# danielSanchezQ/dkg

Hardware: AMD Instinct MI355X
Metric: verified shares/sec (whole node) at n=1024,t=511; full-ceremony wall time (higher is better)
Workload: dtype u32 (GF(2^255-19), Z_l); 1 GPU; one DKG ceremony n=1024, t=511 (share gen + round-2/4 checks + finalise); n=1024, t=511, parallelism=single GPU, verify_streams=2, rounds_2_4_fused=True, degree_split=4, recombination=short lattice multipliers, recombination_addends=affine Niels, stepping_additions=dedicated (complete redo where exceptional)

## Files before the change

dkg_amd/__init__.py:

```python
from ._lib import (ACCEPT, COMPLAINT_IGNORED, COMPLAINT_NO_PHASE3, COMPLAINT_NOT_OWNED, MISSING, REJECT, SELF,
                   SKIPPED, DkgError, lib)
from .api import (Backend, BatchProvenResult, BatchResult, MultiBackend, CeremonyResult, ProvenResult, Environment, ceremony_batch_device,
                  ceremony_batch_full_device, ceremony_batch_verify, ceremony_batch_verify_full, ceremony_batch_verify_full_proven,
                  ceremony_batch_verify_proven, comb_geometry, dealer_coefficients, enc_randomness, env_check, key_comb_choice, merge_verdicts,
                  packed_row_words, pair_eval_shape, receiver_plan, receiver_plan_constants, seat_disclosures, seat_enc_digits, seat_eval_shape, seat_finalise_status, seat_pack,
                  shard_range, shard_rows, split_multipliers)

__all__ = ["Backend", "MultiBackend", "Environment", "CeremonyResult", "BatchResult", "DkgError", "dealer_coefficients", "env_check",
           "ceremony_batch_device", "ceremony_batch_verify", "ceremony_batch_full_device", "ceremony_batch_verify_full", "enc_randomness", "split_multipliers", "lib",
           "shard_range", "shard_rows", "packed_row_words", "key_comb_choice",
           "ceremony_batch_verify_proven", "ceremony_batch_verify_full_proven", "BatchProvenResult",
           "ACCEPT", "REJECT", "SELF", "SKIPPED", "MISSING", "ProvenResult", "COMPLAINT_IGNORED", "COMPLAINT_NO_PHASE3",
           "COMPLAINT_NOT_OWNED", "merge_verdicts", "receiver_plan", "receiver_plan_constants", "pair_eval_shape",
           "comb_geometry", "seat_pack", "seat_finalise_status", "seat_disclosures", "seat_enc_digits", "seat_eval_shape"]
```

dkg_amd/_lib.py:

```python
import ctypes
import os
import sys

HERE = os.path.dirname(os.path.abspath(__file__))
LIB_PATH = os.environ.get("DKG_AMD_LIB", os.path.join(HERE, "libdkg_amd.so"))

DKG_OK = 0
DKG_E_ARG = -1
DKG_E_DECODE = -2
DKG_E_DEVICE = -3
DKG_E_NOMEM = -4
REJECT, ACCEPT, SELF, SKIPPED, MISSING = 0, 1, 2, 3, 4
FIN_OK, FIN_R2_ERROR, FIN_R4_ERROR, FIN_PHASE4_ERROR, FIN_INSUFFICIENT, FIN_PANIC = 0, 1, 2, 3, 4, 5
COMPLAINT_IGNORED, COMPLAINT_NO_PHASE3 = 4, 5
COMPLAINT_NOT_OWNED = -2

_lib = None


class DkgError(RuntimeError):
    def __init__(self, code, msg=""):
        self.code = code
        names = {DKG_E_ARG: "DKG_E_ARG", DKG_E_DECODE: "DKG_E_DECODE", DKG_E_DEVICE: "DKG_E_DEVICE",
                 DKG_E_NOMEM: "DKG_E_NOMEM"}
# ... 211 lines not shown
    L.dkg_dealer_coeffs.argtypes = [u8p, ctypes.c_uint32, sz, sz, sz, p, p]
    L.dkg_scalar_sum_device.argtypes = [p, sz, sz, p, p, p]
    L.dkg_point_sum_device.argtypes = [p, sz, p, p, p]
    L.dkg_share_gen_device.argtypes = [p, sz, sz, sz, p, p, p, p, p, p]
    L.dkg_ceremony_shard_recon_device.argtypes = [p, sz, sz, sz, sz, u8p, u8p, u8p, u8p, p, p,
                                                  ctypes.POINTER(ctypes.c_int32)]
    L.dkg_finalise_parties.argtypes = [p, sz, sz, u8p, u8p, u8p, u8p, u8p, u8p, u8p, p, p, p]
    L.dkg_shard_range.argtypes = [sz, sz, sz, ctypes.POINTER(sz), ctypes.POINTER(sz)]
    L.dkg_shard_range.restype = None
    L.dkg_shard_rows.argtypes = [sz, sz]
    L.dkg_shard_rows.restype = sz
    L.dkg_shard_combine_device.argtypes = [p, sz, sz, sz, p, p, p, p, ctypes.POINTER(ShardOutcome)]
    L.dkg_shard_combine_packed_device.argtypes = [p, sz, sz, sz, p, p, p, p, ctypes.POINTER(ShardOutcome)]
    L.dkg_fixed_base_windows.argtypes = []
    L.dkg_key_comb_windows.argtypes = []
    if hasattr(L, "dkg_comb_geometry"):
        L.dkg_ctx_set_comb_build.argtypes = [p, ctypes.c_int]
        L.dkg_ctx_last_comb_build.argtypes = [p]
        L.dkg_ctx_last_comb_build_ms.argtypes = [p]
        L.dkg_ctx_last_comb_build_ms.restype = ctypes.c_double
        L.dkg_comb_geometry.argtypes = [ctypes.c_int, ctypes.POINTER(ctypes.c_int), ctypes.POINTER(ctypes.c_int),
                                        ctypes.POINTER(ctypes.c_uint32), ctypes.POINTER(ctypes.c_uint32)]
        L.dkg_comb_entries.argtypes = [p, ctypes.c_int, u8p, ctypes.c_int, ctypes.c_uint32, ctypes.c_uint32, p]
    L.dkg_packed_row_words.argtypes = [sz]
    L.dkg_packed_row_words.restype = sz
    L.dkg_decisions_pack_device.argtypes = [p, sz, sz, sz, sz, p, p]
    L.dkg_shard_finalise_device.argtypes = [p, sz, sz, sz, p, p, u8p, ctypes.c_int, p, p, p]
    L.dkg_multi_create.argtypes = [ctypes.POINTER(ctypes.c_int), ctypes.c_int, ctypes.POINTER(p)]
    L.dkg_multi_destroy.argtypes = [p]
    L.dkg_multi_destroy.restype = None
    L.dkg_multi_size.argtypes = [p]
    L.dkg_multi_ctx.argtypes = [p, ctypes.c_int]
    L.dkg_multi_ctx.restype = p
    L.dkg_multi_last_error.argtypes = [p]
    L.dkg_multi_last_error.restype = ctypes.c_char_p
    L.dkg_multi_phase_ms.argtypes = [p, ctypes.c_char_p]
    L.dkg_multi_phase_ms.restype = ctypes.c_double
    L.dkg_multi_env_init.argtypes = [p, sz, sz, u8p, sz, p]
    L.dkg_multi_ceremony_run.argtypes = [p, sz, sz, u8p, u8p, ctypes.POINTER(CeremonyOut)]
    L.dkg_multi_ceremony_run_device.argtypes = [p, sz, sz, ctypes.POINTER(p), ctypes.POINTER(p),
                                                ctypes.POINTER(CeremonyOut)]
    L.dkg_multi_ceremony_verify.argtypes = [p, sz, sz, u8p, u8p, u8p, u8p, ctypes.POINTER(CeremonyOut)]
    L.dkg_multi_ceremony_run_full.argtypes = [p, sz, sz, u8p, u8p, u8p, u8p, u8p, ctypes.POINTER(CeremonyOut)]
    L.dkg_multi_ceremony_run_full_device.argtypes = [p, sz, sz, ctypes.POINTER(p), ctypes.POINTER(p), ctypes.POINTER(p),
                                                     u8p, u8p, ctypes.POINTER(CeremonyOut)]
    L.dkg_multi_ceremony_verify_full.argtypes = [p, sz, sz, u8p, u8p, u8p, u8p, u8p, ctypes.POINTER(CeremonyOut)]
# ... 19 lines not shown
    "dkg_shard_combine_packed_device", "dkg_packed_row_words", "dkg_fixed_base_windows", "dkg_key_comb_windows", "dkg_decisions_pack_device",
    "dkg_shard_finalise_device", "dkg_multi_create", "dkg_multi_destroy", "dkg_multi_size", "dkg_multi_ctx",
    "dkg_multi_last_error", "dkg_multi_phase_ms", "dkg_multi_env_init", "dkg_multi_ceremony_run",
    "dkg_multi_ceremony_run_device", "dkg_multi_ceremony_verify",
    "dkg_member_keys_batch", "dkg_encrypt_shares_batch", "dkg_decrypt_shares_batch", "dkg_ceremony_batch_full_device",
    "dkg_ceremony_batch_verify_full", "dkg_ctx_set_batch_full_chunk",
    "dkg_complaints_prove", "dkg_complaints_verify", "dkg_ctx_set_complaint_eval", "dkg_ceremony_verify_full_complaints",
    "dkg_complaints3_verify", "dkg_ceremony_verify_fetched_proven", "dkg_ceremony_verify_full_proven",
    "dkg_ceremony_batch_verify_proven", "dkg_ceremony_batch_verify_full_proven",
    "dkg_ceremony_shard_full_device", "dkg_ceremony_shard_verify_full_device", "dkg_ctx_set_key_comb",
    "dkg_ctx_last_key_comb", "dkg_key_comb_choice", "dkg_key_comb_constants", "dkg_multi_ceremony_run_full",
    "dkg_multi_ceremony_run_full_device", "dkg_multi_ceremony_verify_full",
    "dkg_ceremony_shard_verify_proven_device", "dkg_ceremony_shard_verify_full_proven_device",
    "dkg_ctx_last_complaint_eval", "dkg_shard_combine_proven_device",
    "dkg_multi_ceremony_verify_proven", "dkg_multi_ceremony_verify_full_proven",
    "dkg_receiver_plan_for", "dkg_receiver_plan_cost_us", "dkg_receiver_plan_constants", "dkg_ctx_set_receiver_chunk",
    "dkg_ctx_set_comb_build", "dkg_ctx_last_comb_build", "dkg_ctx_last_comb_build_ms", "dkg_comb_geometry", "dkg_comb_entries",
    "dkg_ctx_last_receiver_chunk", "dkg_pair_eval_shape", "dkg_commitment_eval_pairs", "dkg_commitment_eval", "dkg_verify_receivers", "dkg_party_round2",
    "dkg_seat_pack", "dkg_commitment_eval_seats", "dkg_verify_seats", "dkg_party_round2_seats",
    "dkg_complaints_verify_ceremonies", "dkg_complaints3_verify_ceremonies", "dkg_party_round3_seats", "dkg_finalise_seats",
    "dkg_seat_finalise_status",
    "dkg_party_round1_seats", "dkg_ctx_set_seat_deal", "dkg_ctx_last_seat_deal", "dkg_seat_enc_digits",
    "dkg_seat_eval_shape", "dkg_seat_eval_constants", "dkg_ctx_set_seat_eval", "dkg_ctx_last_seat_eval",
]
```

dkg_amd/api.py:

```python
import ctypes
from collections.abc import Sequence
from dataclasses import dataclass
from typing import List, Optional

from . import _lib
from ._lib import BatchOut, CeremonyOut, DkgError

CK_DEFAULT = b"Example of a shared string."


def _check(ctx, rc):
    if rc != _lib.DKG_OK:
        msg = _lib.lib().dkg_ctx_last_error(ctx).decode() if ctx else ""
        raise DkgError(rc, msg)


def env_check(threshold: int, nr_members: int) -> None:
    rc = _lib.lib().dkg_env_check(threshold, nr_members)
    if rc != _lib.DKG_OK:
        raise DkgError(rc, f"threshold {threshold} must be < (nr_members + 1) / 2 = {(nr_members + 1) // 2}")


def dealer_coefficients(master: bytes, ceremony: int, d0: int, D: int, t: int):
    N = t + 1
# ... 241 lines not shown
        arr = _carray(ctypes.c_uint32, M, xs)
        out = ctypes.create_string_buffer(32 * max(D * M, 1))
        _check(self._ctx, _lib.lib().dkg_poly_eval_batch(self._ctx, D, N, coeffs, M, arr, out))
        return out.raw[: 32 * D * M]

    def points_valid(self, points: bytes) -> bytes:
        count = len(points) // 32
        out = ctypes.create_string_buffer(max(count, 1))
        _check(self._ctx, _lib.lib().dkg_points_valid_batch(self._ctx, count, points, out))
        return out.raw[:count]

    def share_gen(self, a: bytes, b: bytes, D: int, n: int, t: int):
        N = t + 1
        E, A = ctypes.create_string_buffer(32 * D * N), ctypes.create_string_buffer(32 * D * N)
        s, sp = ctypes.create_string_buffer(32 * D * n), ctypes.create_string_buffer(32 * D * n)
        _check(self._ctx, _lib.lib().dkg_share_gen(self._ctx, D, n, t, a, b, E, A, s, sp))
        return E.raw, A.raw, s.raw, sp.raw

    def share_gen_device(self, D: int, n: int, t: int, d_a: int, d_b: int, d_E: Optional[int], d_A: Optional[int],
                         d_s: int, d_sp: int):
        vp = ctypes.c_void_p
        _check(self._ctx, _lib.lib().dkg_share_gen_device(self._ctx, D, n, t, vp(d_a), vp(d_b), vp(d_E), vp(d_A),
                                                           vp(d_s), vp(d_sp)))

    def verify_pairs(self, n: int, t: int, rnd: int, d0: int, d1: int, C: bytes, s: bytes,
                     s_prime: Optional[bytes] = None) -> bytes:
        dec = ctypes.create_string_buffer(max((d1 - d0) * n, 1))
        _check(self._ctx, _lib.lib().dkg_verify_pairs(self._ctx, n, t, rnd, d0, d1, C, s, s_prime, dec))
        return dec.raw[: (d1 - d0) * n]

    def verify_receiver(self, n: int, t: int, rnd: int, j: int, C: bytes, s_col: bytes,
                        sp_col: Optional[bytes] = None) -> bytes:
        dec = ctypes.create_string_buffer(max(n, 1))
        _check(self._ctx, _lib.lib().dkg_verify_receiver(self._ctx, n, t, rnd, j, C, s_col, sp_col, dec))
        return dec.raw[:n]

    def set_receiver_chunk(self, chunk: int = 0):
        _check(self._ctx, _lib.lib().dkg_ctx_set_receiver_chunk(self._ctx, chunk))

    def last_receiver_chunk(self) -> int:
        return _lib.lib().dkg_ctx_last_receiver_chunk(self._ctx)

    def commitment_eval(self, D: int, t: int, js: Sequence[int], C: bytes):
        M = len(js)
        arr = (ctypes.c_uint32 * max(M, 1))(*js)
        P = ctypes.create_string_buffer(max(32 * M * D, 1))
# ... 751 lines not shown
    v = [ctypes.c_uint32() for _ in range(4)]
    rc = _lib.lib().dkg_seat_pack(n, S, ja, ctypes.byref(v[0]), ctypes.byref(v[1]), ctypes.byref(v[2]), wave_of, slot_of,
                                  ctypes.byref(v[3]))
    if rc != _lib.DKG_OK:
        raise _lib.DkgError(rc, "seat_pack")
    return {"width": v[0].value, "per_wave": v[1].value, "tiles": v[2].value, "wave_of": list(wave_of[:S]),
            "slot_of": list(slot_of[:S]), "waves": v[3].value}


def seat_eval_shape(n: int, t: int, waves: int, x_max: int, chunk: int = 0) -> dict:
    v = [ctypes.c_uint32() for _ in range(3)]
    sb = ctypes.c_uint64()
    L = _lib.lib()
    rc = L.dkg_seat_eval_shape(n, t, waves, x_max, chunk, *[ctypes.byref(x) for x in v], ctypes.byref(sb))
    if rc != _lib.DKG_OK:
        raise _lib.DkgError(rc, "seat_eval_shape")
    c = (ctypes.c_double * 6)()
    L.dkg_seat_eval_constants(c)
    return {"chunk": v[0].value, "chunks": v[1].value, "stages": v[2].value, "scratch_bytes": sb.value,
            "constants": dict(zip(("launch_us", "op_latency_us", "lane_op_us", "serial_op_latency_us",
                                   "chunked_setup_us", "margin"), c))}


def seat_enc_digits(k: int) -> List[int]:
    if k < 0 or k >= 1 << 256:
        raise _lib.DkgError(_lib.DKG_E_ARG, "seat_enc_digits")
    d = (ctypes.c_int8 * 128)()
    w = ctypes.c_int(0)
    rc = _lib.lib().dkg_seat_enc_digits(k.to_bytes(32, "little"), d, ctypes.byref(w))
    if rc != _lib.DKG_OK:
        raise _lib.DkgError(rc, "seat_enc_digits")
    return list(d[: w.value])


def seat_finalise_status(n: int, t: int, p: int, qualified, reconstruct, points: Sequence[int], a_present=None,
                         r2_error: bool = False, r4_error: bool = False):
    mask = lambda x: None if x is None else bytes(bytearray(x))
    idx = ctypes.c_int32(-1)
    rc = _lib.lib().dkg_seat_finalise_status(n, t, p, mask(qualified), mask(reconstruct), mask(a_present),
                                             (ctypes.c_uint32 * max(n, 1))(*points), int(bool(r2_error)),
                                             int(bool(r4_error)), ctypes.byref(idx))
    if rc < 0:
        raise _lib.DkgError(rc, "seat_finalise_status")
    return rc, idx.value


# ... 242 lines not shown
```

dkg_amd/csrc/kernels_decl.inc:

```
namespace dkgk {

void decode_points(const uint32_t* comp, size_t count, uint32_t* ext, size_t stride, uint8_t* ok,
                   hipStream_t stream);
void place_position_major(const uint32_t* src, size_t sstride, size_t D, size_t N, size_t npad, uint32_t* out,
                          hipStream_t stream, int nseg = 1, int seg = 0, size_t L = 0, size_t pstride = 0);
void gather_points(const uint32_t* src, size_t sstride, size_t step, size_t k0, size_t count, uint32_t* dst,
                   size_t dstride, hipStream_t stream);
void decode_position_major(const uint32_t* comp, size_t D, size_t N, size_t npad, uint32_t* out, uint8_t* ok,
                           hipStream_t stream, int nseg = 1, int seg = 0, size_t L = 0, size_t pstride = 0);
void fill_identity(size_t S, uint32_t* out, hipStream_t stream);
void check_both(size_t ndealers, size_t nrecv, size_t dealer0, size_t dealer_base, size_t nmod, const uint32_t* s,
                const uint32_t* sp, const uint32_t* R, const uint32_t* tab_g, const uint32_t* tab_h,
                const uint8_t* dok, uint8_t* dec2, uint8_t* dec4, hipStream_t stream, const uint32_t* scale = nullptr,
                size_t j0 = 0, size_t jn = 0, uint32_t* acc = nullptr);
void encode_points(const uint32_t* ext, size_t stride, size_t count, uint32_t* comp, hipStream_t stream);
void build_comb(const uint32_t* ext, size_t stride, size_t e0, uint32_t* tab, hipStream_t stream, size_t count = 1);
void build_combw(const uint32_t* ext, size_t stride, size_t e0, uint32_t* tab, hipStream_t stream, size_t count = 1);

void commit_position_major(size_t D, size_t N, const uint32_t* a, const uint32_t* b, const uint32_t* tab_g,
                           const uint32_t* tab_h, uint32_t* out, size_t W, size_t L, size_t pstride, uint32_t* A0,
                           size_t A0stride, hipStream_t stream);
void commit(size_t count, const uint32_t* a, const uint32_t* b, const uint32_t* tab_g,
            const uint32_t* tab_h, uint32_t* A_ext, uint32_t* E_ext, hipStream_t stream, size_t stride = 0);
void share_eval(size_t D, size_t n, size_t N, const uint32_t* a, const uint32_t* b, uint32_t* s,
                uint32_t* sp, hipStream_t stream);
void poly_eval(size_t D, size_t N, const uint32_t* coeffs, size_t M, const uint32_t* xs, uint32_t* out,
               hipStream_t stream);

uint32_t* binomial(size_t width, size_t npad, size_t N, const uint32_t* C, uint32_t* e0, uint32_t* e1,
                   hipStream_t stream, size_t pieces = 1, size_t pstride = 0, size_t last_len = 0);
void binom_init(size_t width, size_t npad, size_t N, const uint32_t* C, uint32_t* e0, hipStream_t stream,
                size_t pieces = 1, size_t pstride = 0);
void binom_step(size_t r, size_t width, size_t npad, size_t N, const uint32_t* C, const uint32_t* in, uint32_t* out,
                hipStream_t stream, size_t pieces = 1, size_t pstride = 0, size_t last_len = 0,
                uint32_t* flags = nullptr, size_t col_base = 0, size_t dreal = 0, unsigned gw = 64,
                bool flag_any = false,
                bool nt = false,
                bool il = false);
void binomial_wave_redo(size_t width, size_t npad, size_t N, const uint32_t* C, uint32_t* e, hipStream_t stream,
                        size_t pieces, size_t pstride, size_t last_len, uint32_t* flags, size_t col_base,
                        size_t dreal, unsigned gw);
uint32_t* binomial_wave(size_t width, size_t npad, size_t N, const uint32_t* C, uint32_t* e, hipStream_t stream,
                        size_t pieces = 1, size_t pstride = 0, size_t last_len = 0, uint32_t* eT = nullptr,
                        bool prefetch = false, uint32_t* flags = nullptr, size_t col_base = 0, size_t dreal = 0,
                        unsigned gw = 64);
void binom_step_pair(size_t r, size_t width, size_t npad, size_t N, const uint32_t* C, const uint32_t* in,
                     uint32_t* out, hipStream_t stream, size_t pieces = 1, size_t pstride = 0, size_t last_len = 0);
void to_column_major(size_t width, size_t npad, size_t N, const uint32_t* e, uint32_t* eT, size_t pieces,
// ... 192 lines not shown
```

dkg_amd/csrc/runtime.hip:

```cpp
#include <hip/hip_runtime.h>

#include <cstdio>
#include <cstdlib>
#include <cstring>
#include <algorithm>
#include <array>
#include <iterator>
#include <map>
#include <memory>
#include <optional>
#include <string>
#include <thread>
#include <unordered_map>
#include <unordered_set>
#include <vector>

#include "../../include/dkg_amd.h"
#include "host_crypto.h"
#include "kernels.h"
#include "kernels_ilp.h"
#include "comb_build.h"
#include "seat_finalise.h"
#include "seat_deal.h"

// ... 9 lines not shown
  uint32_t* tab_hw = nullptr;
  uint8_t h[32] = {0};
  bool have_h = false;
  size_t threshold = 0, nr_members = 0;
  hipEvent_t ev[8] = {};
  struct PhaseMark {
    const char* tag;
    int phase;
  };
  std::vector<hipEvent_t> phase_pool;
  std::vector<PhaseMark> phase_marks;
  int receiver_chunk = 0;
  int last_receiver_chunk = 0;
  std::map<std::array<size_t, 4>, dkg_receiver_plan> recv_plans;
  std::map<std::array<size_t, 3>, std::vector<uint32_t>> pair_digits;
  static constexpr int MAX_SUB = 8;
  int nsub = 2;
  hipStream_t sub[MAX_SUB] = {};
  hipEvent_t fork = nullptr, join[MAX_SUB] = {};
  hipStream_t side = nullptr;
  hipEvent_t side_fork = nullptr, shares_done = nullptr, pub_done = nullptr;
  hipEvent_t terms_done = nullptr;
  bool shares_pending = false;
  bool overlap = true;
  int split = 0;
  std::vector<uint8_t> key_tabs_pk;
  std::vector<uint8_t> key_tabs16_pk;
  int key_comb = 0;
  int last_key_comb = 0;
  int seat_deal = 0;
  int last_seat_deal = 0;
  int seat_eval = 0, seat_eval_chunk = 0;
  int last_seat_eval = 0, last_seat_eval_chunk = 0;
  uint8_t fb_base[32] = {0};
  bool fb_valid = false;
  int comb_build = 0;
  int last_comb_build = 0;
  hipEvent_t cb_ev[2] = {};
  int binom_mode = 0;
  int step_mode = 0;
  int check_mode = 0;
  int fe_mode = 0;
  int verify_mode = 0;
  size_t vinv_N = 0;
  size_t fallback_rows = 0;
  int last_split = 1;
// ... 1222 lines not shown
struct Commitments {
  uint32_t *E, *A;
};
Commitments commitment_rows(dkg_ctx* ctx, size_t n, size_t N) {
  uint32_t* EA = buf<uint32_t>(ctx, "cer_EA", 32 * 2 * n * N);
  return {EA, EA + 8 * n * N};
}
Commitments upload_commitments(dkg_ctx* ctx, size_t n, size_t N, const uint8_t* E, const uint8_t* A) {
  const Commitments c = commitment_rows(ctx, n, N);
  h2d(ctx, c.E, E, 32 * n * N);
  h2d(ctx, c.A, A, 32 * n * N);
  return c;
}

void ceremony_times(dkg_ctx* ctx, dkg_ceremony_out* out, bool round1) {
  out->ms_round1 = round1 ? ev_ms(ctx, 0, 1) : 0.0;
  out->ms_round2 = ev_ms(ctx, 1, 2);
  out->ms_round3 = ev_ms(ctx, 2, 3);
  out->ms_round4 = ev_ms(ctx, 3, 4);
  out->ms_finalise = ev_ms(ctx, 4, 5);
  out->ms_total = ev_ms(ctx, 0, 5);
}

void round1_device(dkg_ctx* ctx, size_t D, size_t n, size_t t, const uint32_t* a, const uint32_t* b,
                   uint32_t* Ecomp, uint32_t* Acomp, uint32_t* s, uint32_t* sp, bool encode = true,
                   bool overlap_shares = false) {
  const size_t N = t + 1;
  uint32_t* Aext = buf<uint32_t>(ctx, "Aext", PTB * D * N);
  uint32_t* Eext = buf<uint32_t>(ctx, "Eext", PTB * D * N);
  if (overlap_shares) {
    HCK(hipEventRecord(ctx->side_fork, ctx->stream));
    HCK(hipStreamWaitEvent(ctx->side, ctx->side_fork, 0));
  }
  dkgk::commit(D * N, a, b, ctx->tab_gw, ctx->tab_hw, Aext, Eext, ctx->stream);
  if (encode) {
    dkgk::encode_points(Eext, D * N, D * N, Ecomp, ctx->stream);
    dkgk::encode_points(Aext, D * N, D * N, Acomp, ctx->stream);
  }
  if (overlap_shares) {
    dkgk::share_eval(D, n, N, a, b, s, sp, ctx->side);
    HCK(hipEventRecord(ctx->shares_done, ctx->side));
    ctx->shares_pending = true;
  } else {
    dkgk::share_eval(D, n, N, a, b, s, sp, ctx->stream);
  }
  check_launch(ctx);
}


struct SharesScope {
  dkg_ctx* ctx;
  explicit SharesScope(dkg_ctx* c) : ctx(c) {}
  ~SharesScope() {
    if (ctx->shares_pending) (void)hipStreamWaitEvent(ctx->stream, ctx->shares_done, 0);
    ctx->shares_pending = false;
  }
};

struct ExtScope {
  dkg_ctx* ctx;
  ExtScope(dkg_ctx* c, size_t D, size_t N) : ctx(c) {
    ctx->ext_E = buf<uint32_t>(ctx, "Eext", PTB * D * N);
    ctx->ext_A = buf<uint32_t>(ctx, "Aext", PTB * D * N);
    ctx->ext_stride = D * N;
  }
  ~ExtScope() {
    ctx->ext_E = ctx->ext_A = nullptr;
    ctx->ext_stride = 0;
  }
};

struct BatchRound1 {
  dkg_ctx* ctx;
  BatchRound1(dkg_ctx* c, size_t D, size_t n, size_t t, const uint32_t* a, const uint32_t* b, uint32_t* s,
              uint32_t* sp)
      : ctx(c) {
    const size_t N = t + 1;
    if (deferred()) {
      HCK(hipEventRecord(ctx->side_fork, ctx->stream));
      HCK(hipStreamWaitEvent(ctx->side, ctx->side_fork, 0));
      dkgk::share_eval(D, n, N, a, b, s, sp, ctx->side);
      HCK(hipEventRecord(ctx->shares_done, ctx->side));
      ctx->shares_pending = true;
      ctx->r1_a = a;
      ctx->r1_b = b;
      ctx->r1_D = D;
      ctx->r1_A0 = buf<uint32_t>(ctx, "r1_A0", PTB * D);
    } else {
      round1_device(ctx, D, n, t, a, b, nullptr, nullptr, s, sp, false);
    }
    check_launch(ctx);
  }
  bool deferred() const { return ctx->overlap && ctx->verify_mode == 0; }
  ~BatchRound1() {
    if (ctx->shares_pending) (void)hipStreamWaitEvent(ctx->stream, ctx->shares_done, 0);
    ctx->r1_a = ctx->r1_b = nullptr;
    ctx->r1_D = 0;
    ctx->r1_A0 = nullptr;
    ctx->shares_pending = false;
  }
};

struct BatchProven {
  const uint8_t* a_ok = nullptr;
// ... 1589 lines not shown
    round1_device(ctx, D, n, t, da, db, Ec, Ac, ds, dsp);
    if (E) d2h(ctx, E, Ec, 32 * D * N);
    if (A) d2h(ctx, A, Ac, 32 * D * N);
    if (s) d2h(ctx, s, ds, 32 * D * n);
    if (s_prime) d2h(ctx, s_prime, dsp, 32 * D * n);
    sync(ctx);
    return DKG_OK;
  });
}

int dkg_share_gen_device(dkg_ctx* ctx, size_t D, size_t n, size_t t, const void* d_a, const void* d_b, void* d_E,
                         void* d_A, void* d_s, void* d_s_prime) {
  return guarded(ctx, [&] {
    int rc = need_env(ctx);
    if (rc) return rc;
    if (!d_a || !d_b || !d_s || !d_s_prime) return DKG_E_ARG;
    if (D == 0) return DKG_OK;
    const size_t N = t + 1;
    uint32_t* Ec = d_E ? (uint32_t*)d_E : buf<uint32_t>(ctx, "sgd_E", 32 * D * N);
    uint32_t* Ac = d_A ? (uint32_t*)d_A : buf<uint32_t>(ctx, "sgd_A", 32 * D * N);
    round1_device(ctx, D, n, t, (const uint32_t*)d_a, (const uint32_t*)d_b, Ec, Ac, (uint32_t*)d_s,
                  (uint32_t*)d_s_prime, d_E || d_A);
    sync(ctx);
    return DKG_OK;
  });
}

int dkg_verify_pairs(dkg_ctx* ctx, size_t n, size_t t, int round, size_t d0, size_t d1, const uint8_t* C,
                     const uint8_t* s, const uint8_t* s_prime, uint8_t* decision) {
  return guarded(ctx, [&] {
    if ((round != 2 && round != 4) || d1 < d0 || d1 > n) return DKG_E_ARG;
    if (round == 2) {
      int rc = need_env(ctx);
      if (rc) return rc;
      if (!s_prime) return DKG_E_ARG;
    }
    const size_t D = d1 - d0, N = t + 1;
    if (D == 0) return DKG_OK;
    uint32_t* Cc = buf<uint32_t>(ctx, "vp_C", 32 * D * N);
    h2d(ctx, Cc, C, 32 * D * N);
    uint32_t* ds = upload_scalars(ctx, "vp_s", s, D * n);
    uint32_t* dsp = round == 2 ? upload_scalars(ctx, "vp_sp", s_prime, D * n) : nullptr;
    uint8_t* dec = buf<uint8_t>(ctx, "vp_dec", D * n);
    verify_one(ctx, n, t, round, D, d0, Cc, ds, dsp, dec, false);
    d2h(ctx, decision, dec, D * n);
    sync(ctx);
// ... 811 lines not shown
                             const void* d_dec4_g, void* d_dec2, void* d_dec4, dkg_shard_outcome* out) {
  return guarded(ctx, [&] {
    if (!out || !d_dec2_g || !d_dec4_g || !world_size || world_size > n || dkg_env_check(t, n) != DKG_OK)
      return DKG_E_ARG;
    const size_t R = dkg_shard_rows(n, world_size);
    return shard_combine(ctx, n, t, d_dec2, d_dec4, out, [&](uint8_t* dec2, uint8_t* dec4) {
      dkgk::compact_ranks(n, world_size, R, n, d_dec2_g, dec2, ctx->stream);
      dkgk::compact_ranks(n, world_size, R, n, d_dec4_g, dec4, ctx->stream);
    });
  });
}

size_t dkg_packed_row_words(size_t n) { return (n + 31) / 32 + 1; }

int dkg_fixed_base_windows(void) { return dkgk::fixed_base_windows(); }
int dkg_key_comb_windows(void) { return dkgk::key_comb_windows(); }

int dkg_ctx_set_key_comb(dkg_ctx* ctx, int mode) {
  if (!ctx || mode < 0 || mode > 2) return DKG_E_ARG;
  ctx->key_comb = mode;
  return DKG_OK;
}
int dkg_ctx_last_key_comb(const dkg_ctx* ctx) { return ctx ? ctx->last_key_comb : 0; }

int dkg_ctx_set_seat_deal(dkg_ctx* ctx, int mode) {
  if (!ctx || mode < 0 || mode > 2) return DKG_E_ARG;
  ctx->seat_deal = mode;
  return DKG_OK;
}
int dkg_ctx_last_seat_deal(const dkg_ctx* ctx) { return ctx ? ctx->last_seat_deal : 0; }

int dkg_ctx_set_seat_eval(dkg_ctx* ctx, int mode, int chunk) {
  if (!ctx || mode < 0 || mode > 2 || chunk < 0 || (mode != 2 && chunk != 0)) return DKG_E_ARG;
  ctx->seat_eval = mode;
  ctx->seat_eval_chunk = chunk;
  return DKG_OK;
}
int dkg_ctx_last_seat_eval(const dkg_ctx* ctx, int* chunk) {
  if (chunk) *chunk = ctx ? ctx->last_seat_eval_chunk : 0;
  return ctx ? ctx->last_seat_eval : 0;
}

int dkg_ctx_set_comb_build(dkg_ctx* ctx, int mode) {
  if (!ctx || mode < 0 || mode > 2) return DKG_E_ARG;
  ctx->comb_build = mode;
  ctx->fb_valid = false;
// ... 1972 lines not shown
```

include/dkg_amd.h:

```cpp
#ifndef DKG_AMD_H
#define DKG_AMD_H
#include <stddef.h>
#include <stdint.h>

#ifdef __cplusplus
extern "C" {
#endif

#define DKG_OK 0
#define DKG_E_ARG (-1)
#define DKG_E_DECODE (-2)
#define DKG_E_DEVICE (-3)
#define DKG_E_NOMEM (-4)

#define DKG_REJECT 0
#define DKG_ACCEPT 1
#define DKG_SELF 2
#define DKG_SKIPPED 3
#define DKG_MISSING 4

typedef struct dkg_ctx dkg_ctx;

int dkg_ctx_create(int device, dkg_ctx **out);
void dkg_ctx_destroy(dkg_ctx *ctx);
// ... 30 lines not shown
int dkg_device_count(void);
int dkg_ctx_clock_probe(dkg_ctx *ctx, unsigned iters, double *sclk_mhz, double *busy_ms);
int dkg_device_pci_bus_id(int device, char *buf, int len);

int dkg_env_init(dkg_ctx *ctx, size_t threshold, size_t nr_members, const uint8_t *ck_bytes, size_t ck_len,
                 uint8_t h_out[32]);
int dkg_env_check(size_t threshold, size_t nr_members);

int dkg_msm_batch(dkg_ctx *ctx, size_t B, size_t N, const uint8_t *scalars, const uint8_t *points, uint8_t *out);
int dkg_fixed_base_batch(dkg_ctx *ctx, const uint8_t base[32], size_t count, const uint8_t *scalars, uint8_t *out);
int dkg_poly_eval_batch(dkg_ctx *ctx, size_t D, size_t N, const uint8_t *coeffs, size_t M, const uint32_t *xs,
                        uint8_t *out);
int dkg_points_valid_batch(dkg_ctx *ctx, size_t count, const uint8_t *points, uint8_t *ok);

int dkg_share_gen(dkg_ctx *ctx, size_t D, size_t n, size_t t, const uint8_t *a, const uint8_t *b, uint8_t *E,
                  uint8_t *A, uint8_t *s, uint8_t *s_prime);
int dkg_share_gen_device(dkg_ctx *ctx, size_t D, size_t n, size_t t, const void *d_a, const void *d_b, void *d_E,
                         void *d_A, void *d_s, void *d_s_prime);

int dkg_verify_pairs(dkg_ctx *ctx, size_t n, size_t t, int round, size_t d0, size_t d1, const uint8_t *C,
                     const uint8_t *s, const uint8_t *s_prime, uint8_t *decision);
int dkg_verify_receiver(dkg_ctx *ctx, size_t n, size_t t, int round, size_t j, const uint8_t *C, const uint8_t *s,
                        const uint8_t *s_prime, uint8_t *decision);

typedef struct {
  uint32_t chunk;
  uint32_t stages;
  uint32_t arity[16];
  uint8_t mult[16][32];
} dkg_receiver_plan;
int dkg_receiver_plan_for(size_t n, size_t t, uint32_t x, int chunk, dkg_receiver_plan *out);
double dkg_receiver_plan_cost_us(size_t n, size_t t, uint32_t x, const dkg_receiver_plan *p);
void dkg_receiver_plan_constants(double c[5]);
int dkg_ctx_set_receiver_chunk(dkg_ctx *ctx, int chunk);
int dkg_ctx_last_receiver_chunk(const dkg_ctx *ctx);
int dkg_commitment_eval(dkg_ctx *ctx, size_t D, size_t t, size_t M, const uint32_t *js, const uint8_t *C,
                        uint8_t *P, uint8_t *ok);
int dkg_pair_eval_shape(size_t t, int chunk, uint32_t *L, uint32_t *lanes, uint32_t *stages);
int dkg_commitment_eval_pairs(dkg_ctx *ctx, size_t D, size_t t, size_t count, const uint32_t *rows,
                              const uint32_t *js, const uint8_t *C, uint8_t *P, uint8_t *ok);
int dkg_verify_receivers(dkg_ctx *ctx, size_t n, size_t t, int round, size_t M, const uint32_t *js, const uint8_t *C,
                         const uint8_t *s, const uint8_t *s_prime, const uint8_t *qualified, uint8_t *decision);
int dkg_party_round2(dkg_ctx *ctx, size_t n, size_t t, size_t j, const uint8_t *E, const uint8_t *e1, const uint8_t *ct,
                     const uint8_t sk[32], const uint8_t *w, uint8_t *s_out, uint8_t *sp_out, uint8_t *dec,
                     int32_t *complaints, uint8_t *r2_error, uint8_t *proofs);

// ... 310 lines not shown
```

Baseline: 13.69 million verified shares/s.

## Add finite-difference stepping route for share evaluation with cost-model selection

Adds a new share-evaluation kernel. Each dealer polynomial is converted to a difference form, and the polynomial is stepped across consecutive receiver indices with 9-word additions (periodic folding) instead of a Horner multiply chain per receiver. Long polynomials are split into pieces, one wavefront each, recombined with precomputed powers through LDS. A host-side cost model picks Horner or stepping and the lanes-per-piece count by default. This trades many modular multiplications for additions and DPP lane shifts, at the cost of an extra powers kernel, LDS traffic and a hand-tuned cost model that may misroute.

```diff
diff --git a/dkg_amd/__init__.py b/dkg_amd/__init__.py
--- a/dkg_amd/__init__.py
+++ b/dkg_amd/__init__.py
@@ -4,7 +4,7 @@
                   ceremony_batch_full_device, ceremony_batch_verify, ceremony_batch_verify_full, ceremony_batch_verify_full_proven,
                   ceremony_batch_verify_proven, comb_geometry, dealer_coefficients, enc_randomness, env_check, key_comb_choice, merge_verdicts,
                   packed_row_words, pair_eval_shape, receiver_plan, receiver_plan_constants, seat_disclosures, seat_enc_digits, seat_eval_shape, seat_finalise_status, seat_pack,
-                  shard_range, shard_rows, split_multipliers)
+                  shard_range, shard_rows, share_route, share_steps_shape, split_multipliers)
 
 __all__ = ["Backend", "MultiBackend", "Environment", "CeremonyResult", "BatchResult", "DkgError", "dealer_coefficients", "env_check",
            "ceremony_batch_device", "ceremony_batch_verify", "ceremony_batch_full_device", "ceremony_batch_verify_full", "enc_randomness", "split_multipliers", "lib",
@@ -12,4 +12,5 @@
            "ceremony_batch_verify_proven", "ceremony_batch_verify_full_proven", "BatchProvenResult",
            "ACCEPT", "REJECT", "SELF", "SKIPPED", "MISSING", "ProvenResult", "COMPLAINT_IGNORED", "COMPLAINT_NO_PHASE3",
            "COMPLAINT_NOT_OWNED", "merge_verdicts", "receiver_plan", "receiver_plan_constants", "pair_eval_shape",
-           "comb_geometry", "seat_pack", "seat_finalise_status", "seat_disclosures", "seat_enc_digits", "seat_eval_shape"]
+           "comb_geometry", "seat_pack", "seat_finalise_status", "seat_disclosures", "seat_enc_digits", "seat_eval_shape",
+           "share_route", "share_steps_shape"]
diff --git a/dkg_amd/_lib.py b/dkg_amd/_lib.py
--- a/dkg_amd/_lib.py
+++ b/dkg_amd/_lib.py
@@ -257,6 +257,18 @@
         L.dkg_comb_geometry.argtypes = [ctypes.c_int, ctypes.POINTER(ctypes.c_int), ctypes.POINTER(ctypes.c_int),
                                         ctypes.POINTER(ctypes.c_uint32), ctypes.POINTER(ctypes.c_uint32)]
         L.dkg_comb_entries.argtypes = [p, ctypes.c_int, u8p, ctypes.c_int, ctypes.c_uint32, ctypes.c_uint32, p]
+    if hasattr(L, "dkg_share_route_for"):
+        L.dkg_share_route_for.argtypes = [sz, sz, sz, ctypes.c_int, ctypes.POINTER(ctypes.c_int)]
+        L.dkg_share_route_cost_us.argtypes = [sz, sz, sz, ctypes.c_int, ctypes.c_int]
+        L.dkg_share_route_cost_us.restype = ctypes.c_double
+        L.dkg_share_route_constants.argtypes = [ctypes.POINTER(ctypes.c_double)]
+        L.dkg_share_route_constants.restype = None
+        L.dkg_ctx_set_share_eval.argtypes = [p, ctypes.c_int]
+        L.dkg_ctx_set_share_ppl.argtypes = [p, ctypes.c_int]
+        L.dkg_ctx_last_share_eval.argtypes = [p, ctypes.POINTER(ctypes.c_int)]
+        L.dkg_share_steps_shape.argtypes = [ctypes.POINTER(ctypes.c_uint32)]
+        L.dkg_share_steps_shape.restype = None
+        L.dkg_share_eval_device.argtypes = [p, sz, sz, sz, p, p, p, p, ctypes.POINTER(ctypes.c_double)]
     L.dkg_packed_row_words.argtypes = [sz]
     L.dkg_packed_row_words.restype = sz
     L.dkg_decisions_pack_device.argtypes = [p, sz, sz, sz, sz, p, p]
@@ -322,4 +334,6 @@
     "dkg_seat_finalise_status",
     "dkg_party_round1_seats", "dkg_ctx_set_seat_deal", "dkg_ctx_last_seat_deal", "dkg_seat_enc_digits",
     "dkg_seat_eval_shape", "dkg_seat_eval_constants", "dkg_ctx_set_seat_eval", "dkg_ctx_last_seat_eval",
+    "dkg_share_route_for", "dkg_share_route_cost_us", "dkg_share_route_constants", "dkg_ctx_set_share_eval",
+    "dkg_ctx_set_share_ppl", "dkg_ctx_last_share_eval", "dkg_share_steps_shape", "dkg_share_eval_device",
 ]
diff --git a/dkg_amd/api.py b/dkg_amd/api.py
--- a/dkg_amd/api.py
+++ b/dkg_amd/api.py
@@ -287,6 +287,22 @@
         vp = ctypes.c_void_p
         _check(self._ctx, _lib.lib().dkg_share_gen_device(self._ctx, D, n, t, vp(d_a), vp(d_b), vp(d_E), vp(d_A),
                                                            vp(d_s), vp(d_sp)))
+
+    def share_eval_device(self, D: int, n: int, t: int, d_a: int, d_b: int, d_s: int, d_sp: int) -> float:
+        vp = ctypes.c_void_p
+        ms = ctypes.c_double(0.0)
+        _check(self._ctx, _lib.lib().dkg_share_eval_device(self._ctx, D, n, t, vp(d_a), vp(d_b), vp(d_s), vp(d_sp),
+                                                            ctypes.byref(ms)))
+        return ms.value
+
+    def set_share_eval(self, mode: int = 0, ppl: int = 0):
+        _check(self._ctx, _lib.lib().dkg_ctx_set_share_eval(self._ctx, mode))
+        _check(self._ctx, _lib.lib().dkg_ctx_set_share_ppl(self._ctx, ppl))
+
+    def last_share_eval(self) -> tuple:
+        c = ctypes.c_int(0)
+        route = _lib.lib().dkg_ctx_last_share_eval(self._ctx, ctypes.byref(c))
+        return route, c.value
 
     def verify_pairs(self, n: int, t: int, rnd: int, d0: int, d1: int, C: bytes, s: bytes,
                      s_prime: Optional[bytes] = None) -> bytes:
@@ -1084,6 +1100,29 @@
                                    "chunked_setup_us", "margin"), c))}
 
 
+def share_route(D: int, n: int, t: int, mode: int = 0) -> dict:
+    L = _lib.lib()
+    ppl = ctypes.c_int(0)
+    route = L.dkg_share_route_for(D, n, t, mode, ctypes.byref(ppl))
+    if route < 0:
+        raise _lib.DkgError(route, "share_route")
+    best = ctypes.c_int(0)
+    L.dkg_share_route_for(D, n, t, 2, ctypes.byref(best))
+    c = (ctypes.c_double * 10)()
+    L.dkg_share_route_constants(c)
+    return {"route": route, "ppl": ppl.value, "horner_us": L.dkg_share_route_cost_us(D, n, t, 1, 0),
+            "steps_us": L.dkg_share_route_cost_us(D, n, t, 2, best.value) if best.value else -1.0,
+            "constants": dict(zip(("launch_us", "horner_us", "horner_chain_us", "build_us", "step_us_ppl1",
+                                   "step_us_ppl2", "step_us_ppl4", "chain_row_us", "chain_step_us",
+                                   "chain_block_us"), c))}
+
+
+def share_steps_shape() -> dict:
+    v = (ctypes.c_uint32 * 5)()
+    _lib.lib().dkg_share_steps_shape(v)
+    return dict(zip(("words", "folded_bits", "fold", "block", "max_pieces"), v))
+
+
 def seat_enc_digits(k: int) -> List[int]:
     if k < 0 or k >= 1 << 256:
         raise _lib.DkgError(_lib.DKG_E_ARG, "seat_enc_digits")
diff --git a/dkg_amd/csrc/kernels_decl.inc b/dkg_amd/csrc/kernels_decl.inc
--- a/dkg_amd/csrc/kernels_decl.inc
+++ b/dkg_amd/csrc/kernels_decl.inc
@@ -24,6 +24,11 @@
             const uint32_t* tab_h, uint32_t* A_ext, uint32_t* E_ext, hipStream_t stream, size_t stride = 0);
 void share_eval(size_t D, size_t n, size_t N, const uint32_t* a, const uint32_t* b, uint32_t* s,
                 uint32_t* sp, hipStream_t stream);
+bool share_steps_covers(size_t n, size_t N, int ppl);
+size_t share_steps_power_words(size_t n, size_t N, int ppl);
+bool share_steps(size_t D, size_t n, size_t N, int ppl, const uint32_t* a, const uint32_t* b, uint32_t* pw,
+                 uint32_t* s, uint32_t* sp, hipStream_t stream);
+void share_steps_shape(uint32_t* words, uint32_t* folded_bits, uint32_t* fold, uint32_t* block, uint32_t* max_pieces);
 void poly_eval(size_t D, size_t N, const uint32_t* coeffs, size_t M, const uint32_t* xs, uint32_t* out,
                hipStream_t stream);
 
diff --git a/dkg_amd/csrc/runtime.hip b/dkg_amd/csrc/runtime.hip
--- a/dkg_amd/csrc/runtime.hip
+++ b/dkg_amd/csrc/runtime.hip
@@ -55,6 +55,9 @@
   hipEvent_t side_fork = nullptr, shares_done = nullptr, pub_done = nullptr;
   hipEvent_t terms_done = nullptr;
   bool shares_pending = false;
+  int share_eval = 0;
+  int share_ppl = 0;
+  int last_share_eval = 0, last_share_ppl = 0;
   bool overlap = true;
   int split = 0;
   std::vector<uint8_t> key_tabs_pk;
@@ -1323,6 +1326,25 @@
   out->ms_total = ev_ms(ctx, 0, 5);
 }
 
+void share_eval_routed(dkg_ctx* ctx, size_t D, size_t n, size_t N, const uint32_t* a, const uint32_t* b, uint32_t* s,
+                       uint32_t* sp, hipStream_t stream) {
+  if (!D || !n) return;
+  int ppl = 0;
+  const int route = dkg_share_route_for(D, n, N - 1, ctx->share_eval, &ppl);
+  if (route == 2 && ctx->share_ppl && dkgk::share_steps_covers(n, N, ctx->share_ppl)) ppl = ctx->share_ppl;
+  if (route == 2) {
+    uint32_t* pw = buf<uint32_t>(ctx, "share_pw", 4 * dkgk::share_steps_power_words(n, N, ppl));
+    if (!dkgk::share_steps(D, n, N, ppl, a, b, pw, s, sp, stream)) {
+      ctx->err = "share_steps: the route rule chose a shape the kernel does not cover";
+      throw Fail{DKG_E_ARG};
+    }
+  } else {
+    dkgk::share_eval(D, n, N, a, b, s, sp, stream);
+  }
+  ctx->last_share_eval = route == 2 ? 2 : 1;
+  ctx->last_share_ppl = route == 2 ? ppl : 0;
+}
+
 void round1_device(dkg_ctx* ctx, size_t D, size_t n, size_t t, const uint32_t* a, const uint32_t* b,
                    uint32_t* Ecomp, uint32_t* Acomp, uint32_t* s, uint32_t* sp, bool encode = true,
                    bool overlap_shares = false) {
@@ -1339,11 +1361,11 @@
     dkgk::encode_points(Aext, D * N, D * N, Acomp, ctx->stream);
   }
   if (overlap_shares) {
-    dkgk::share_eval(D, n, N, a, b, s, sp, ctx->side);
+    share_eval_routed(ctx, D, n, N, a, b, s, sp, ctx->side);
     HCK(hipEventRecord(ctx->shares_done, ctx->side));
     ctx->shares_pending = true;
   } else {
-    dkgk::share_eval(D, n, N, a, b, s, sp, ctx->stream);
+    share_eval_routed(ctx, D, n, N, a, b, s, sp, ctx->stream);
   }
   check_launch(ctx);
 }
@@ -1380,7 +1402,7 @@
     if (deferred()) {
       HCK(hipEventRecord(ctx->side_fork, ctx->stream));
       HCK(hipStreamWaitEvent(ctx->side, ctx->side_fork, 0));
-      dkgk::share_eval(D, n, N, a, b, s, sp, ctx->side);
+      share_eval_routed(ctx, D, n, N, a, b, s, sp, ctx->side);
       HCK(hipEventRecord(ctx->shares_done, ctx->side));
       ctx->shares_pending = true;
       ctx->r1_a = a;
@@ -3016,6 +3038,23 @@
     round1_device(ctx, D, n, t, (const uint32_t*)d_a, (const uint32_t*)d_b, Ec, Ac, (uint32_t*)d_s,
                   (uint32_t*)d_s_prime, d_E || d_A);
     sync(ctx);
+    return DKG_OK;
+  });
+}
+
+int dkg_share_eval_device(dkg_ctx* ctx, size_t D, size_t n, size_t t, const void* d_a, const void* d_b, void* d_s,
+                          void* d_s_prime, double* device_ms) {
+  return guarded(ctx, [&] {
+    if (!d_a || !d_b || !d_s || !d_s_prime) return DKG_E_ARG;
+    if (device_ms) *device_ms = 0.0;
+    if (D == 0 || n == 0) return DKG_OK;
+    HCK(hipEventRecord(ctx->ev[6], ctx->stream));
+    share_eval_routed(ctx, D, n, t + 1, (const uint32_t*)d_a, (const uint32_t*)d_b, (uint32_t*)d_s,
+                      (uint32_t*)d_s_prime, ctx->stream);
+    HCK(hipEventRecord(ctx->ev[7], ctx->stream));
+    check_launch(ctx);
+    sync(ctx);
+    if (device_ms) *device_ms = ev_ms(ctx, 6, 7);
     return DKG_OK;
   });
 }
@@ -3873,6 +3912,24 @@
   return DKG_OK;
 }
 int dkg_ctx_last_key_comb(const dkg_ctx* ctx) { return ctx ? ctx->last_key_comb : 0; }
+
+int dkg_ctx_set_share_eval(dkg_ctx* ctx, int mode) {
+  if (!ctx || mode < 0 || mode > 2) return DKG_E_ARG;
+  ctx->share_eval = mode;
+  return DKG_OK;
+}
+int dkg_ctx_set_share_ppl(dkg_ctx* ctx, int ppl) {
+  if (!ctx || (ppl != 0 && ppl != 1 && ppl != 2 && ppl != 4)) return DKG_E_ARG;
+  ctx->share_ppl = ppl;
+  return DKG_OK;
+}
+int dkg_ctx_last_share_eval(const dkg_ctx* ctx, int* ppl) {
+  if (ppl) *ppl = ctx ? ctx->last_share_ppl : 0;
+  return ctx ? ctx->last_share_eval : 0;
+}
+void dkg_share_steps_shape(uint32_t shape[5]) {
+  if (shape) dkgk::share_steps_shape(shape, shape + 1, shape + 2, shape + 3, shape + 4);
+}
 
 int dkg_ctx_set_seat_deal(dkg_ctx* ctx, int mode) {
   if (!ctx || mode < 0 || mode > 2) return DKG_E_ARG;
diff --git a/dkg_amd/csrc/share_route.cpp b/dkg_amd/csrc/share_route.cpp
--- /dev/null
+++ b/dkg_amd/csrc/share_route.cpp
@@ -0,0 +1,62 @@
+#include "../../include/dkg_amd.h"
+
+namespace {
+
+constexpr size_t SR_BLOCK = 64, SR_MAX_PIECES = 8;
+
+size_t pieces_of(size_t N, int ppl) { return (N + SR_BLOCK * (size_t)ppl - 1) / (SR_BLOCK * (size_t)ppl); }
+
+bool covers(size_t n, size_t N, int ppl) {
+  return (ppl == 1 || ppl == 2 || ppl == 4) && n >= SR_BLOCK && n < ((size_t)1 << 32) && N >= 1 &&
+         pieces_of(N, ppl) <= SR_MAX_PIECES;
+}
+
+const double SR_LAUNCH_US = 7.1, SR_HORNER_US = 1.3e-6, SR_HORNER_CHAIN_US = 0.25, SR_BUILD_US = 7.75e-7,
+             SR_STEP_US[3] = {1.016e-6, 6.9e-7, 6.8e-7}, SR_CHAIN_ROW_US = 0.1, SR_CHAIN_STEP_US = 0.1,
+             SR_CHAIN_BLOCK_US = 8.0;
+
+}
+
+extern "C" {
+
+void dkg_share_route_constants(double c[10]) {
+  if (!c) return;
+  c[0] = SR_LAUNCH_US, c[1] = SR_HORNER_US, c[2] = SR_HORNER_CHAIN_US, c[3] = SR_BUILD_US;
+  c[4] = SR_STEP_US[0], c[5] = SR_STEP_US[1], c[6] = SR_STEP_US[2];
+  c[7] = SR_CHAIN_ROW_US, c[8] = SR_CHAIN_STEP_US, c[9] = SR_CHAIN_BLOCK_US;
+}
+
+double dkg_share_route_cost_us(size_t D, size_t n, size_t t, int route, int ppl) {
+  const size_t N = t + 1;
+  if (!D || !n || N < 1) return -1.0;
+  const double pairs = 2.0 * (double)D * (double)n;
+  if (route == 1) {
+    const double thr = pairs * (double)N * SR_HORNER_US, chain = (double)N * SR_HORNER_CHAIN_US;
+    return SR_LAUNCH_US + (thr > chain ? thr : chain);
+  }
+  if (route != 2 || !covers(n, N, ppl)) return -1.0;
+  const double L = (double)(SR_BLOCK * (size_t)ppl), U = (double)pieces_of(N, ppl);
+  const double rows = (double)N < L ? (double)N : L;
+  const double thr = pairs * U * L * (rows / (double)n * SR_BUILD_US + SR_STEP_US[ppl == 1 ? 0 : (ppl == 2 ? 1 : 2)]);
+  const double chain = rows * (double)ppl * SR_CHAIN_ROW_US + (double)n * (double)ppl * SR_CHAIN_STEP_US +
+                       (double)((n + SR_BLOCK - 1) / SR_BLOCK) * SR_CHAIN_BLOCK_US;
+  return SR_LAUNCH_US * (U > 1 ? 2.0 : 1.0) + (thr > chain ? thr : chain);
+}
+
+int dkg_share_route_for(size_t D, size_t n, size_t t, int mode, int* ppl) {
+  if (ppl) *ppl = 0;
+  if (mode < 0 || mode > 2 || !D || !n) return DKG_E_ARG;
+  if (mode == 1) return 1;
+  int best = 0;
+  double best_us = 0.0;
+  for (int p = 1; p <= 4; p *= 2) {
+    const double us = dkg_share_route_cost_us(D, n, t, 2, p);
+    if (us >= 0.0 && (!best || us < best_us)) best = p, best_us = us;
+  }
+  if (!best) return 1;
+  if (mode == 0 && dkg_share_route_cost_us(D, n, t, 1, 0) <= best_us) return 1;
+  if (ppl) *ppl = best;
+  return 2;
+}
+
+}
diff --git a/dkg_amd/csrc/share_steps.hip b/dkg_amd/csrc/share_steps.hip
--- /dev/null
+++ b/dkg_amd/csrc/share_steps.hip
@@ -0,0 +1,248 @@
+#include "kernels.h"
+#include "points.h"
+
+namespace dkgk {
+
+namespace {
+
+constexpr int SS_WORDS = 9;
+constexpr int SS_FOLDED_BITS = 254;
+constexpr int SS_BLOCK = 64;
+constexpr int SS_FOLD = 32;
+static_assert(SS_FOLDED_BITS + SS_FOLD <= 32 * SS_WORDS, "an accumulator would overflow before its fold");
+static_assert(SS_FOLDED_BITS + 2 * SS_FOLD > 32 * SS_WORDS && SS_BLOCK % SS_FOLD == 0,
+              "the fold interval is the largest divisor of the block within the bound");
+constexpr int SS_MAX_PIECES = 8;
+constexpr int SS_CAP_WORDS = SS_BLOCK * SS_WORDS, SS_PROD_WORDS = 8 * SS_BLOCK;
+
+DKG_DEV void ss_fold(uint32_t (&v)[SS_WORDS]) {
+  const uint32_t h0 = (v[7] >> 28) | (v[8] << 4), h1 = v[8] >> 28;
+  uint32_t p[6];
+  uint64_t c = 0;
+#pragma unroll
+  for (int i = 0; i < 4; i++) {
+    c += (uint64_t)h0 * sc_const::DELTA[i];
+    p[i] = (uint32_t)c;
+    c >>= 32;
+  }
+  p[4] = (uint32_t)c;
+  c = 0;
+#pragma unroll
+  for (int i = 0; i < 4; i++) {
+    c += (uint64_t)h1 * sc_const::DELTA[i] + p[i + 1];
+    p[i + 1] = (uint32_t)c;
+    c >>= 32;
+  }
+  p[5] = (uint32_t)c;
+  int64_t d = 0;
+#pragma unroll
+  for (int i = 0; i < 8; i++) {
+    const uint32_t lo = i < 7 ? v[i] : (v[7] & 0x0fffffffu);
+    d += (int64_t)lo + sc_const::L[i] - (i < 6 ? p[i] : 0u);
+    v[i] = (uint32_t)d;
+    d >>= 32;
+  }
+  v[8] = 0;
+}
+
+DKG_DEV void ss_add(uint32_t (&x)[SS_WORDS], const uint32_t (&y)[SS_WORDS]) {
+  unsigned c = 0;
+#pragma unroll
+  for (int i = 0; i < SS_WORDS; i++) x[i] = __builtin_addc(x[i], y[i], c, &c);
+}
+
+DKG_DEV uint32_t ss_from_next(uint32_t x) {
+  return (uint32_t)__builtin_amdgcn_update_dpp(0, (int)x, 0x130 , 0xf, 0xf, true);
+}
+DKG_DEV uint32_t ss_from_prev(uint32_t x) {
+  return (uint32_t)__builtin_amdgcn_update_dpp(0, (int)x, 0x138 , 0xf, 0xf, true);
+}
+
+DKG_DEV void ss_reduce9(sc& r, const uint32_t (&x)[9]) {
+  const uint32_t q = (x[7] >> 28) | (x[8] << 4);
+  uint32_t t[5];
+  uint64_t c = 0;
+#pragma unroll
+  for (int i = 0; i < 4; i++) {
+    c += (uint64_t)q * sc_const::DELTA[i];
+    t[i] = (uint32_t)c;
+    c >>= 32;
+  }
+  t[4] = (uint32_t)c;
+  unsigned bw = 0;
+#pragma unroll
+  for (int i = 0; i < 8; i++)
+    r.v[i] = __builtin_subc(i < 7 ? x[i] : (x[7] & 0x0fffffffu), i < 5 ? t[i] : 0u, bw, &bw);
+  const uint32_t mask = 0u - bw;
+  unsigned cy = 0;
+#pragma unroll
+  for (int i = 0; i < 8; i++) r.v[i] = __builtin_addc(r.v[i], sc_const::L[i] & mask, cy, &cy);
+}
+
+DKG_DEV void ss_build_item(sc& r, const sc& x, const sc& y, uint32_t m, const sc& c) {
+  uint32_t s[8], w[9];
+  unsigned cy = 0;
+#pragma unroll
+  for (int i = 0; i < 8; i++) s[i] = __builtin_addc(x.v[i], y.v[i], cy, &cy);
+  uint64_t acc = 0;
+#pragma unroll
+  for (int i = 0; i < 8; i++) {
+    acc += (uint64_t)s[i] * m + c.v[i];
+    w[i] = (uint32_t)acc;
+    acc >>= 32;
+  }
+  w[8] = (uint32_t)acc;
+  ss_reduce9(r, w);
+}
+
+__global__ __launch_bounds__(64) void k_share_powers(size_t n, uint32_t U, uint32_t logL, uint32_t* __restrict__ pw) {
+  const size_t j = (size_t)blockIdx.x * blockDim.x + threadIdx.x;
+  if (j >= n) return;
+  sc x, y, p;
+  sc_zero(x);
+  x.v[0] = (uint32_t)(j + 1);
+#pragma unroll
+  for (int i = 0; i < 8; i++) y.v[i] = sc_const::RR[i];
+  sc_mont_mul(y, x, y);
+#pragma unroll 1
+  for (uint32_t k = 0; k < logL; k++) sc_mont_mul(y, y, y);
+  p = y;
+#pragma unroll 1
+  for (uint32_t u = 1; u < U; u++) {
+    st_words8(pw + 8 * ((size_t)(u - 1) * n + j), p.v);
+    sc_mont_mul(p, p, y);
+  }
+}
+
+template <int PPL>
+__global__ __launch_bounds__(64 * SS_MAX_PIECES) void k_share_steps(size_t D, size_t n, size_t N,
+                                                                     const uint32_t* __restrict__ a,
+                                                                     const uint32_t* __restrict__ b,
+                                                                     const uint32_t* __restrict__ pw,
+                                                                     uint32_t* __restrict__ s,
+                                                                     uint32_t* __restrict__ sp) {
+  extern __shared__ uint32_t ss_lds[];
+  constexpr uint32_t L = 64 * PPL;
+  const size_t q = blockIdx.x;
+  const uint32_t u = (uint32_t)__builtin_amdgcn_readfirstlane((int)(threadIdx.x >> 6));
+  const uint32_t U = (uint32_t)(blockDim.x >> 6), lane = threadIdx.x & 63u;
+  const uint32_t* coef = q < D ? a + 8 * q * N : b + 8 * (q - D) * N;
+  uint32_t* out = q < D ? s + 8 * q * n : sp + 8 * (q - D) * n;
+  uint32_t* cap = ss_lds + (size_t)u * SS_CAP_WORDS;
+  uint32_t* prod = ss_lds + (size_t)U * SS_CAP_WORDS;
+
+  sc e[PPL];
+#pragma unroll
+  for (int p = 0; p < PPL; p++) sc_zero(e[p]);
+  const size_t g0 = (size_t)u * L;
+  const uint32_t len = (uint32_t)(N - g0 < L ? N - g0 : L);
+#pragma unroll 1
+  for (uint32_t k = len; k-- > 0;) {
+    sc c, prev;
+    sc_load(c, coef + 8 * (g0 + k));
+#pragma unroll
+    for (int i = 0; i < 8; i++) {
+      prev.v[i] = ss_from_prev(e[PPL - 1].v[i]);
+      c.v[i] = lane == 0 ? c.v[i] : 0u;
+    }
+    sc zero;
+    sc_zero(zero);
+#pragma unroll
+    for (int p = PPL - 1; p > 0; p--) ss_build_item(e[p], e[p - 1], e[p], PPL * lane + p, zero);
+    ss_build_item(e[0], prev, e[0], PPL * lane, c);
+  }
+
+  uint32_t d[PPL][SS_WORDS];
+#pragma unroll
+  for (int p = 0; p < PPL; p++)
+#pragma unroll
+    for (int i = 0; i < SS_WORDS; i++) d[p][i] = i < 8 ? e[p].v[i] : 0u;
+
+#pragma unroll 1
+  for (size_t j0 = 0; j0 < n; j0 += SS_BLOCK) {
+    const uint32_t cnt = (uint32_t)(n - j0 < SS_BLOCK ? n - j0 : SS_BLOCK);
+    sc y;
+    sc_zero(y);
+    if (u > 0 && lane < cnt) sc_load(y, pw + 8 * ((size_t)(u - 1) * n + j0 + lane));
+#pragma unroll 1
+    for (uint32_t i0 = 0; i0 < cnt; i0 += SS_FOLD) {
+      const uint32_t i1 = i0 + SS_FOLD < cnt ? i0 + SS_FOLD : cnt;
+#pragma unroll 1
+      for (uint32_t i = i0; i < i1; i++) {
+        uint32_t nb[SS_WORDS];
+#pragma unroll
+        for (int w = 0; w < SS_WORDS; w++) nb[w] = ss_from_next(d[0][w]);
+#pragma unroll
+        for (int p = 0; p + 1 < PPL; p++) ss_add(d[p], d[p + 1]);
+        ss_add(d[PPL - 1], nb);
+        if (lane == 0) {
+#pragma unroll
+          for (int w = 0; w < SS_WORDS; w++) cap[i * SS_WORDS + w] = d[0][w];
+        }
+      }
+#pragma unroll
+      for (int p = 0; p < PPL; p++) ss_fold(d[p]);
+    }
+    __syncthreads();
+    if (lane < cnt) {
+      uint32_t v[SS_WORDS];
+#pragma unroll
+      for (int w = 0; w < SS_WORDS; w++) v[w] = cap[lane * SS_WORDS + w];
+      ss_fold(v);
+      sc r;
+      ss_reduce9(r, v);
+      if (u > 0) sc_mont_mul(r, r, y);
+#pragma unroll
+      for (int w = 0; w < 8; w++) prod[((size_t)u * 8 + w) * SS_BLOCK + lane] = r.v[w];
+    }
+    __syncthreads();
+    if (u == 0 && lane < cnt) {
+      uint32_t v[9];
+      uint64_t acc = 0;
+#pragma unroll
+      for (int w = 0; w < 8; w++) {
+        for (uint32_t k = 0; k < U; k++) acc += prod[((size_t)k * 8 + w) * SS_BLOCK + lane];
+        v[w] = (uint32_t)acc;
+        acc >>= 32;
+      }
+      v[8] = (uint32_t)acc;
+      sc r;
+      ss_reduce9(r, v);
+      st_words8(out + 8 * (j0 + lane), r.v);
+    }
+  }
+}
+
+uint32_t pieces_of(size_t N, int ppl) { return (uint32_t)((N + 64 * (size_t)ppl - 1) / (64 * (size_t)ppl)); }
+
+}
+
+bool share_steps_covers(size_t n, size_t N, int ppl) {
+  if (ppl != 1 && ppl != 2 && ppl != 4) return false;
+  return n >= SS_BLOCK && n < ((size_t)1 << 32) && N >= 1 && pieces_of(N, ppl) <= (uint32_t)SS_MAX_PIECES;
+}
+
+size_t share_steps_power_words(size_t n, size_t N, int ppl) {
+  return share_steps_covers(n, N, ppl) ? 8 * n * (size_t)(pieces_of(N, ppl) - 1) : 0;
+}
+
+void share_steps_shape(uint32_t* words, uint32_t* folded_bits, uint32_t* fold, uint32_t* block, uint32_t* max_pieces) {
+  *words = SS_WORDS, *folded_bits = SS_FOLDED_BITS, *fold = SS_FOLD, *block = SS_BLOCK, *max_pieces = SS_MAX_PIECES;
+}
+
+bool share_steps(size_t D, size_t n, size_t N, int ppl, const uint32_t* a, const uint32_t* b, uint32_t* pw,
+                 uint32_t* s, uint32_t* sp, hipStream_t stream) {
+  if (!share_steps_covers(n, N, ppl) || 2 * D > 0x7fffffffu) return false;
+  if (!D) return true;
+  const uint32_t U = pieces_of(N, ppl);
+  const uint32_t logL = ppl == 1 ? 6 : (ppl == 2 ? 7 : 8);
+  if (U > 1) hipLaunchKernelGGL(k_share_powers, dim3((unsigned)((n + 63) / 64)), dim3(64), 0, stream, n, U, logL, pw);
+  const dim3 grid((unsigned)(2 * D)), block(64 * U);
+  const size_t lds = (size_t)U * (SS_CAP_WORDS + SS_PROD_WORDS) * 4;
+  if (ppl == 1) hipLaunchKernelGGL(k_share_steps<1>, grid, block, lds, stream, D, n, N, a, b, pw, s, sp);
+  else if (ppl == 2) hipLaunchKernelGGL(k_share_steps<2>, grid, block, lds, stream, D, n, N, a, b, pw, s, sp);
+  else hipLaunchKernelGGL(k_share_steps<4>, grid, block, lds, stream, D, n, N, a, b, pw, s, sp);
+  return true;
+}
+
+}
diff --git a/include/dkg_amd.h b/include/dkg_amd.h
--- a/include/dkg_amd.h
+++ b/include/dkg_amd.h
@@ -76,6 +76,16 @@
                      const uint8_t *s, const uint8_t *s_prime, uint8_t *decision);
 int dkg_verify_receiver(dkg_ctx *ctx, size_t n, size_t t, int round, size_t j, const uint8_t *C, const uint8_t *s,
                         const uint8_t *s_prime, uint8_t *decision);
+
+int dkg_share_route_for(size_t D, size_t n, size_t t, int mode, int *ppl);
+double dkg_share_route_cost_us(size_t D, size_t n, size_t t, int route, int ppl);
+void dkg_share_route_constants(double c[10]);
+int dkg_ctx_set_share_eval(dkg_ctx *ctx, int mode);
+int dkg_ctx_set_share_ppl(dkg_ctx *ctx, int ppl);
+int dkg_ctx_last_share_eval(const dkg_ctx *ctx, int *ppl);
+int dkg_share_eval_device(dkg_ctx *ctx, size_t D, size_t n, size_t t, const void *d_a, const void *d_b, void *d_s,
+                          void *d_s_prime, double *device_ms);
+void dkg_share_steps_shape(uint32_t shape[5]);
 
 typedef struct {
   uint32_t chunk;
```

After: 13.81 million verified shares/s (median of 6 runs). No clear change (+0.8%).
